# annegnx/PnP-Flow

Measured on AMD Instinct MI355X. Metric: restored images/sec, higher is better.
Workload: dtype f32-equivalent (f16 hi+lo split operands, 3 x f16 MFMA per product, f32 accumulate); 1 GPU; CelebA-shaped 256x256 box-inpainting (half-size 40, sigma 0.05) pnp_flow B=32/GPU 100x5 (the configuration BASELINE.json's metric is quoted on; main.py:132-136 at 256^2); image=256x256x3, batch_per_gpu=32, global_batch=32, steps_pnp=100, num_samples=5, weights=synthetic seed 0 (no checkpoint offline), hipgraph=True, unet_batch=160, parallelism=dp1 (contiguous shards of the global batch, no data-path collective)

## Files before the change

pnpflow_amd/csrc/conv_mfma16.hip:

```cpp
#include <cstdlib>
#include "pp_common.h"

namespace pf {

typedef float f32x16 __attribute__((ext_vector_type(16)));
typedef _Float16 f16x8 __attribute__((ext_vector_type(8)));
typedef _Float16 f16x4 __attribute__((ext_vector_type(4)));

__device__ __forceinline__ float silu_fast16(float x) { return x * __builtin_amdgcn_rcpf(1.0f + __expf(-x)); }

constexpr int conv16_lb(int MT, int WM, int KC) { return ((MT == 4 && WM == 2 && KC == 16) || (KC != 64 && ((MT == 4 && WM == 1) || (MT == 2 && WM == 4)))) ? 3 : 1; }

template <int MT, int NT, int WM, int WN, int S, int UP, int KC, bool GNB = false, int TERMS = 3>
__global__ __launch_bounds__(256, conv16_lb(MT, WM, KC)) void conv_mfma16_kernel(const ConvParams p) {
    constexpr int ROW = (TERMS == 3 ? KC : KC / 2) + 4;
    constexpr int KQ = KC / 4, KH = KC / 2, KS = KC / 16;
    constexpr int TH = 2 * MT * WM, TW = 16;
    constexpr int HALO = KC == 64 ? 0 : 1;
    constexpr int PH = (TH - 1) * S + 1 + 2 * HALO, PW = (TW - 1) * S + 1 + 2 * HALO, PP = PH * PW;
    constexpr int RS = ((PW * ROW + 63) / 64) * 64;
    constexpr int BN = WN * NT * 32;
    constexpr int A_F4 = PP * KQ, A_PER = (A_F4 + 255) / 256;
    static_assert(WM * WN == 4, "4 waves per workgroup");

    extern __shared__ __attribute__((aligned(16))) char smem_raw[];
    uint32_t* s_patch = reinterpret_cast<uint32_t*>(smem_raw);
    constexpr int EPI = 4 * 32 * 36 + WM * BN * 2;
    float* s_sc = reinterpret_cast<float*>(s_patch + (PH * RS > EPI ? PH * RS : EPI));
    float* s_sh = s_sc + ((p.gn_C + 3) & ~3);

    const int tiles_x = (p.W + TW - 1) / TW, tiles_y = (p.H + TH - 1) / TH;
    int bid, nb;
    if (p.xcd_map) {
        const int NBk = gridDim.y == 1 ? (p.Cout + BN - 1) / BN : 1;
        const int total = gridDim.x;
        const int work = (blockIdx.x & 7) * (total >> 3) + (blockIdx.x >> 3);
        bid = work / NBk; nb = work % NBk;
    } else {
        bid = blockIdx.x; nb = blockIdx.y;
    }
    const int tx = bid % tiles_x; bid /= tiles_x;
    const int ty = bid % tiles_y;
    const int b = bid / tiles_y;
    const int oy0 = ty * TH, ox0 = tx * TW, n0 = nb * BN;
    const int tid = threadIdx.x, lane = tid & 63, wave = tid >> 6, hi = lane >> 5, l31 = lane & 31;
    const int wm = wave % WM, wn = wave / WM;
    const int Hv = UP ? 2 * p.Hs : p.Hs, Wv = UP ? 2 * p.Ws : p.Ws;
    const int qi = tid % KQ, q4 = qi * 4;
    float seg_scale[3], seg_inv[3];
#pragma unroll
    for (int i = 0; i < 3; ++i) { seg_scale[i] = p.scale != nullptr ? p.scale[8 * b + i] : 1.0f; seg_inv[i] = p.scale != nullptr ? p.scale[8 * b + 4 + i] : 1.0f; }

    int a_pix[A_PER];
#pragma unroll
    for (int i = 0; i < A_PER; ++i) {
        const int idx = tid + i * 256;
        a_pix[i] = -1;
        if (idx < A_F4) {
            const int pix = idx / KQ;
            const int py = pix / PW, px = pix % PW;
            const int gy = oy0 * S - HALO + py, gx = ox0 * S - HALO + px;
            if (gy >= 0 && gy < Hv && gx >= 0 && gx < Wv && !(UP == 2 && ((gy | gx) & 1))) {
                const int sy = UP ? (gy >> 1) : gy, sx = UP ? (gx >> 1) : gx;
                a_pix[i] = (b * p.Hs + sy) * (p.src_row_pitch > 0 ? p.src_row_pitch : p.Ws) + sx;
            }
        }
    }

    float4 ra[A_PER];
    auto prefetch = [&](int si, int ch) {
        const ConvSeg& sg = p.seg[si];
        const int c = min(ch * KC + q4, sg.C - 4);
        const float* base = sg.src + sg.coff + c;
#pragma unroll
        for (int i = 0; i < A_PER; ++i) ra[i] = *reinterpret_cast<const float4*>(base + (size_t)max(a_pix[i], 0) * sg.cstride);
    };
    auto store_lds = [&](int si, int ch) {
        const ConvSeg& sg = p.seg[si];
        const int c = ch * KC + q4;
        const bool cok = c < sg.C;
        float4 sc = make_float4(1.f, 1.f, 1.f, 1.f), sh = make_float4(0.f, 0.f, 0.f, 0.f);
        if (sg.xform != 0 && cok) {
            sc = *reinterpret_cast<const float4*>(s_sc + sg.gn_off + c);
            sh = *reinterpret_cast<const float4*>(s_sh + sg.gn_off + c);
        }
        const float a_scale = si == 0 ? seg_scale[0] : (si == 1 ? seg_scale[1] : seg_scale[2]);
#pragma unroll
        for (int i = 0; i < A_PER; ++i) {
            if (tid + i * 256 < A_F4) {
                const int a_p = (tid + i * 256) / KQ;
                const int a_lds = (a_p / PW) * RS + (a_p % PW) * ROW + qi * 2;
                float4 v = ra[i];
                if (sg.xform != 0) {
                    v.x = v.x * sc.x + sh.x; v.y = v.y * sc.y + sh.y;
                    v.z = v.z * sc.z + sh.z; v.w = v.w * sc.w + sh.w;
                    if (sg.xform == 2) {
                        v.x = silu_fast16(v.x); v.y = silu_fast16(v.y); v.z = silu_fast16(v.z); v.w = silu_fast16(v.w);
                    }
                }
                v.x *= a_scale; v.y *= a_scale; v.z *= a_scale; v.w *= a_scale;
                if (!(cok && a_pix[i] >= 0)) v = make_float4(0.f, 0.f, 0.f, 0.f);
                if constexpr (TERMS == 3) {
                    uint2 h, l;
                    split4_pp(v, h.x, h.y, l.x, l.y);
                    *reinterpret_cast<uint2*>(s_patch + a_lds) = h;
                    *reinterpret_cast<uint2*>(s_patch + a_lds + KH) = l;
                } else {
                    f16x4 h;
                    h[0] = (_Float16)v.x; h[1] = (_Float16)v.y; h[2] = (_Float16)v.z; h[3] = (_Float16)v.w;
                    *reinterpret_cast<f16x4*>(s_patch + a_lds) = h;
                }
            }
        }
    };

    constexpr int GNP = 4;
    float csc[GNP], csh[GNP];
    {
        const float* cb = p.coef + (size_t)b * 2 * p.coef_stride;
#pragma unroll
        for (int i = 0; i < GNP; ++i) {
            csc[i] = 0.f; csh[i] = 0.f;
            if (i * 256 < p.gn_C) {
                const int c = min(tid + i * 256, p.gn_C - 1);
                csc[i] = cb[c]; csh[i] = cb[p.coef_stride + c];
            }
        }
    }
    prefetch(0, 0);
#pragma unroll
    for (int i = 0; i < GNP; ++i) {
        const int c = tid + i * 256;
        if (c < p.gn_C) { s_sc[c] = csc[i]; s_sh[c] = csh[i]; }
    }

    f32x16 acc[MT][NT];
#pragma unroll
    for (int mt = 0; mt < MT; ++mt)
#pragma unroll
        for (int nt = 0; nt < NT; ++nt)
#pragma unroll
            for (int r = 0; r < 16; ++r) acc[mt][nt][r] = 0.f;

    const int prow = l31 >> 4, pcol = l31 & 15;
    const int nbase = n0 + wn * NT * 32 + l31;
    int nclamp[NT];
#pragma unroll
    for (int nt = 0; nt < NT; ++nt) nclamp[nt] = min(nbase + nt * 32, p.Cout - 1);

    auto load_b = [&](const ConvSeg& sg, int ch, int s, uint4 (&dh)[NT], uint4 (&dl)[NT]) {
        const int tap = s / KS, j = s % KS;
        const size_t kidx = ((size_t)ch * KS + j) * sg.taps + tap;
        const uint4* wp = reinterpret_cast<const uint4*>(sg.w16) + kidx * ((size_t)p.Cout * 4) + hi;
#pragma unroll
        for (int nt = 0; nt < NT; ++nt) { dh[nt] = wp[(size_t)nclamp[nt] * 2]; if constexpr (TERMS == 3) dl[nt] = wp[(size_t)p.Cout * 2 + (size_t)nclamp[nt] * 2]; else dl[nt] = dh[nt]; }
    };

    int si = 0, ch = 0;
    while (true) {
        const ConvSeg& sg = p.seg[si];
        if (ch == 0 && si > 0) {
            const float ratio = (si == 1 ? seg_scale[1] * seg_inv[0] : seg_scale[2] * seg_inv[1]);
            if (ratio != 1.0f)
            {
#pragma unroll
                for (int mt = 0; mt < MT; ++mt)
#pragma unroll
                    for (int nt = 0; nt < NT; ++nt)
#pragma unroll
                        for (int r = 0; r < 16; ++r) acc[mt][nt][r] *= ratio;
            }
        }
        __syncthreads();
        store_lds(si, ch);
        __syncthreads();
        int nsi = si, nch = ch + 1;
        if (nch * KC >= sg.C) { nsi = si + 1; nch = 0; }
        const bool more = nsi < p.nseg;

        const int nsteps = sg.taps * KS;
        uint4 bh0[NT], bl0[NT], bh1[NT], bl1[NT], bh2[NT], bl2[NT];
        load_b(sg, ch, 0, bh0, bl0); load_b(sg, ch, min(1, nsteps - 1), bh1, bl1);
        if (more) prefetch(nsi, nch);

        auto k_step = [&](int s, uint4 (&ch_)[NT], uint4 (&cl_)[NT], uint4 (&nh_)[NT], uint4 (&nl_)[NT]) {
            load_b(sg, ch, min(s + 2, nsteps - 1), nh_, nl_);
            __builtin_amdgcn_sched_barrier(0);
            const int tap = s / KS, j = s % KS;
            const int ky = sg.taps == 9 ? tap / 3 : (sg.taps == 4 ? (tap >> 1) + sg.oy : HALO), kx = sg.taps == 9 ? tap % 3 : (sg.taps == 4 ? (tap & 1) + sg.ox : HALO);
            f16x8 ah[MT], al[MT];
#pragma unroll
            for (int mt = 0; mt < MT; ++mt) {
                const int poff = (((wm * MT + mt) * 2 + prow) * S + ky) * RS + (pcol * S + kx) * ROW;
                ah[mt] = *reinterpret_cast<const f16x8*>(s_patch + poff + j * 8 + hi * 4);
                if constexpr (TERMS == 3) al[mt] = *reinterpret_cast<const f16x8*>(s_patch + poff + KH + j * 8 + hi * 4); else al[mt] = ah[mt];
            }
            if constexpr (!(MT == 4 && WM == 1)) __builtin_amdgcn_sched_barrier(0);
            if constexpr (TERMS == 3) {
#pragma unroll
            for (int mt = 0; mt < MT; ++mt)
#pragma unroll
                for (int nt = 0; nt < NT; ++nt)
                    acc[mt][nt] = __builtin_amdgcn_mfma_f32_32x32x16_f16(al[mt], *reinterpret_cast<const f16x8*>(&ch_[nt]), acc[mt][nt], 0, 0, 0);
#pragma unroll
            for (int mt = 0; mt < MT; ++mt)
#pragma unroll
                for (int nt = 0; nt < NT; ++nt)
                    acc[mt][nt] = __builtin_amdgcn_mfma_f32_32x32x16_f16(ah[mt], *reinterpret_cast<const f16x8*>(&cl_[nt]), acc[mt][nt], 0, 0, 0);
            }
#pragma unroll
            for (int mt = 0; mt < MT; ++mt)
#pragma unroll
                for (int nt = 0; nt < NT; ++nt)
                    acc[mt][nt] = __builtin_amdgcn_mfma_f32_32x32x16_f16(ah[mt], *reinterpret_cast<const f16x8*>(&ch_[nt]), acc[mt][nt], 0, 0, 0);
        };
        __builtin_amdgcn_s_setprio(2);
        int s = 0;
        for (; s + 3 <= nsteps; s += 3) {
            k_step(s, bh0, bl0, bh2, bl2); k_step(s + 1, bh1, bl1, bh0, bl0); k_step(s + 2, bh2, bl2, bh1, bl1);
        }
        if (nsteps - s >= 1) k_step(s, bh0, bl0, bh2, bl2);
        if (nsteps - s == 2) k_step(s + 1, bh1, bl1, bh0, bl0);
        __builtin_amdgcn_s_setprio(0);
        if (!more) break;
        si = nsi; ch = nch;
    }

    __syncthreads();
    constexpr int TP = 36;
    float* s_tr = reinterpret_cast<float*>(s_patch) + wave * (32 * TP);
    float* s_red = reinterpret_cast<float*>(s_patch) + 4 * 32 * TP;
    const float oscale = p.out_scale * (1.0f / 256.0f) * (p.nseg == 1 ? seg_inv[0] : (p.nseg == 2 ? seg_inv[1] : seg_inv[2]));
    const int cq = lane & 7;
#pragma unroll
    for (int nt = 0; nt < NT; ++nt) {
        const int ncol = n0 + (wn * NT + nt) * 32;
        const int n = ncol + l31;
        const float add = (p.addvec != nullptr && n < p.Cout) ? p.addvec[(size_t)b * p.addvec_bs + n] : 0.f;
        const int n4 = ncol + cq * 4;
        const bool nok4 = n4 < p.Cout;
        float s1[4] = {0.f, 0.f, 0.f, 0.f}, s2[4] = {0.f, 0.f, 0.f, 0.f};
        float4 g_mu, g_rs, g_ga, g_be;
        if constexpr (GNB) {
            const int gc = p.gnb_coff + min(n4, p.Cout - 4);
            g_mu = *reinterpret_cast<const float4*>(p.gnb_mu + (size_t)b * p.gnb_Ct + gc);
            g_rs = *reinterpret_cast<const float4*>(p.gnb_rs + (size_t)b * p.gnb_Ct + gc);
            g_ga = *reinterpret_cast<const float4*>(p.gnb_gamma + gc);
            g_be = *reinterpret_cast<const float4*>(p.gnb_beta + gc);
        }
        constexpr int RG = (MT >= 2 && WN != 4) ? 2 : 1;
        float4 rv[RG][4];
        float4 xv[GNB ? RG : 1][4];
#pragma unroll
        for (int mt = 0; mt < MT; ++mt) {
            if constexpr (GNB) {
                if (mt % RG == 0) {
#pragma unroll
                    for (int g = 0; g < RG; ++g)
#pragma unroll
                        for (int i = 0; i < 4; ++i) {
                            const int px = (lane >> 3) + 8 * i;
                            const int oy = min(oy0 + (wm * MT + mt + g) * 2 + (px >> 4), p.H - 1), ox = min(ox0 + (px & 15), p.W - 1);
                            const size_t pix = ((size_t)b * p.H + oy) * p.W + ox;
                            xv[g][i] = *reinterpret_cast<const float4*>(p.gnb_x + pix * p.gnb_xstride + min(n4, p.Cout - 4));
                        }
                }
            }
            if (mt % RG == 0 && p.residual != nullptr) {
#pragma unroll
                for (int g = 0; g < RG; ++g)
#pragma unroll
                    for (int i = 0; i < 4; ++i) {
                        const int px = (lane >> 3) + 8 * i;
                        const int oy = min(oy0 + (wm * MT + mt + g) * 2 + (px >> 4), p.H - 1), ox = min(ox0 + (px & 15), p.W - 1);
                        const size_t pix = ((size_t)b * p.H + oy) * (p.dst_row_pitch > 0 ? p.dst_row_pitch : p.W) + ox;
                        rv[g][i] = *reinterpret_cast<const float4*>(p.residual + pix * p.res_cstride + min(n4, p.Cout - 4));
                    }
            }
#pragma unroll
            for (int r = 0; r < 16; ++r) {
                const int row = (r & 3) + 8 * (r >> 2) + 4 * hi;
                s_tr[row * TP + l31] = acc[mt][nt][r] * oscale + add;
            }
            __builtin_amdgcn_fence(__ATOMIC_RELEASE, "workgroup");
            __builtin_amdgcn_wave_barrier();
            __builtin_amdgcn_fence(__ATOMIC_ACQUIRE, "workgroup");
#pragma unroll
            for (int i = 0; i < 4; ++i) {
                const int px = (lane >> 3) + 8 * i;
                const int oy = oy0 + (wm * MT + mt) * 2 + (px >> 4), ox = ox0 + (px & 15);
                float4 v = *reinterpret_cast<const float4*>(s_tr + px * TP + cq * 4);
                if (nok4 && oy < p.H && ox < p.W) {
                    const size_t pix = ((size_t)b * p.H + oy) * (p.dst_row_pitch > 0 ? p.dst_row_pitch : p.W) + ox;
                    if (p.residual != nullptr) {
                        const float rsc = p.res_scale;
                        v.x = fmaf(rv[mt % RG][i].x, rsc, v.x); v.y = fmaf(rv[mt % RG][i].y, rsc, v.y); v.z = fmaf(rv[mt % RG][i].z, rsc, v.z); v.w = fmaf(rv[mt % RG][i].w, rsc, v.w);
                    }
                    if constexpr (GNB) {
                        const float4 xx = xv[mt % RG][i];
                        float d[4] = {v.x, v.y, v.z, v.w};
                        const float xs[4] = {xx.x, xx.y, xx.z, xx.w}, mm[4] = {g_mu.x, g_mu.y, g_mu.z, g_mu.w}, rr[4] = {g_rs.x, g_rs.y, g_rs.z, g_rs.w};
                        const float gg[4] = {g_ga.x, g_ga.y, g_ga.z, g_ga.w}, bb[4] = {g_be.x, g_be.y, g_be.z, g_be.w};
#pragma unroll
                        for (int j = 0; j < 4; ++j) {
                            const float yh = (xs[j] - mm[j]) * rr[j];
                            if (p.gnb_silu) {
                                const float u = yh * gg[j] + bb[j];
                                const float sg = __builtin_amdgcn_rcpf(1.0f + __expf(-u));
                                d[j] *= sg * (1.0f + u * (1.0f - sg));
                            }
                            d[j] *= gg[j];
                            s1[j] += d[j]; s2[j] += d[j] * yh;
                        }
                        *reinterpret_cast<float4*>(p.out + pix * p.out_cstride + n4) = make_float4(d[0], d[1], d[2], d[3]);
                    } else {
                    *reinterpret_cast<float4*>(p.out + pix * p.out_cstride + n4) = (p.pack_from_p1 != 0 && n4 >= p.pack_from_p1 - 1) ? pack_hilo4(v) : v;
                    s1[0] += v.x; s1[1] += v.y; s1[2] += v.z; s1[3] += v.w;
                    s2[0] += v.x * v.x; s2[1] += v.y * v.y; s2[2] += v.z * v.z; s2[3] += v.w * v.w;
                    }
                }
            }
            __builtin_amdgcn_fence(__ATOMIC_RELEASE, "workgroup");
            __builtin_amdgcn_wave_barrier();
            __builtin_amdgcn_fence(__ATOMIC_ACQUIRE, "workgroup");
        }
        if (GNB || p.stats_out != nullptr) {
#pragma unroll
            for (int j = 0; j < 4; ++j) {
#pragma unroll
                for (int o = 8; o < 64; o <<= 1) { s1[j] += __shfl_xor(s1[j], o); s2[j] += __shfl_xor(s2[j], o); }
            }
            if (lane < 8) {
#pragma unroll
                for (int j = 0; j < 4; ++j) {
                    const int col = (wn * NT + nt) * 32 + cq * 4 + j;
                    s_red[(wm * BN + col) * 2] = s1[j]; s_red[(wm * BN + col) * 2 + 1] = s2[j];
                }
            }
        }
    }
    if (GNB || p.stats_out != nullptr) {
        __syncthreads();
        for (int t = tid; t < BN * 2; t += 256) {
            const int col = t >> 1, which = t & 1;
            float tot = 0.f;
#pragma unroll
            for (int w = 0; w < WM; ++w) tot += s_red[(w * BN + col) * 2 + which];
            const int n = n0 + col;
            if (n < p.Cout) {
                if constexpr (GNB) unsafeAtomicAdd(p.gnb_sum + ((size_t)b * p.gnb_Ct + p.gnb_coff + n) * 2 + which, (double)tot);
                else unsafeAtomicAdd(p.stats_out + ((size_t)b * p.Cout + n) * 2 + which, (double)tot);
            }
        }
    }
}

template <int MT, int NT, int WM, int WN, int S, int UP, int KC, int TERMS>
static hipError_t launch_cfg16(const ConvParams& p, hipStream_t stream) {
    constexpr int ROW = (TERMS == 3 ? KC : KC / 2) + 4;
    constexpr int TH = 2 * MT * WM, TW = 16;
    constexpr int HALO = KC == 64 ? 0 : 1;
    constexpr int PH = (TH - 1) * S + 1 + 2 * HALO, PW = (TW - 1) * S + 1 + 2 * HALO;
    constexpr int RS = ((PW * ROW + 63) / 64) * 64;
    constexpr int BN = WN * NT * 32;
    constexpr int EPI = 4 * 32 * 36 + WM * BN * 2;
    const size_t lds = (size_t)((PH * RS > EPI ? PH * RS : EPI) + 2 * ((p.gn_C + 3) & ~3)) * 4;
    const int tiles = p.B * ((p.H + TH - 1) / TH) * ((p.W + TW - 1) / TW);
    dim3 grid(tiles, (p.Cout + BN - 1) / BN);
    ConvParams pp = p; pp.xcd_map = 0;
    if (((long)grid.x * grid.y) % 8 == 0) { pp.xcd_map = 1; grid = dim3(grid.x * grid.y, 1); }
    if constexpr (S == 1 && UP == 0) {
        if (p.gnb_x != nullptr) {
            static unsigned long long attr_set_g = 0ull;
            auto kg = conv_mfma16_kernel<MT, NT, WM, WN, S, UP, KC, true, TERMS>;
            { hipError_t e = set_max_dynamic_lds_once(reinterpret_cast<const void*>(kg), attr_set_g, 160 * 1024); if (e != hipSuccess) return e; }
            hipLaunchKernelGGL(kg, grid, dim3(256), lds, stream, pp);
            return hipGetLastError();
        }
    }
    if (p.gnb_x != nullptr) return hipErrorInvalidValue;
    static unsigned long long attr_set = 0ull;
    auto kern = conv_mfma16_kernel<MT, NT, WM, WN, S, UP, KC, false, TERMS>;
    { hipError_t e = set_max_dynamic_lds_once(reinterpret_cast<const void*>(kern), attr_set, 160 * 1024); if (e != hipSuccess) return e; }
    hipLaunchKernelGGL(kern, grid, dim3(256), lds, stream, pp);
    return hipGetLastError();
}

static long wg_count16(const ConvParams& p, int TH, int BN) {
    return (long)p.B * ((p.H + TH - 1) / TH) * ((p.W + 15) / 16) * ((p.Cout + BN - 1) / BN);
}

template <int S, int UP, int KC, int TERMS>
static hipError_t launch_sel16(const ConvParams& p, hipStream_t stream) {
    constexpr long MIN_WGS = KC == 64 ? 1024 : 512;
    if constexpr (S == 1) {
        if (p.Cout <= 32) {
            return launch_cfg16<2, 1, 4, 1, S, UP, KC, TERMS>(p, stream);
        }
        if (p.Cout <= 64) {
            if (wg_count16(p, 16, 64) >= MIN_WGS) return launch_cfg16<4, 1, 2, 2, S, UP, KC, TERMS>(p, stream);
            if (wg_count16(p, 8, 64) >= MIN_WGS) return launch_cfg16<2, 1, 2, 2, S, UP, KC, TERMS>(p, stream);
            return launch_cfg16<1, 1, 2, 2, S, UP, KC, TERMS>(p, stream);
        }
        if (wg_count16(p, 8, 128) >= MIN_WGS) return launch_cfg16<4, 1, 1, 4, S, UP, KC, TERMS>(p, stream);
        if (wg_count16(p, 4, 128) >= MIN_WGS) return launch_cfg16<2, 1, 1, 4, S, UP, KC, TERMS>(p, stream);
        return launch_cfg16<1, 1, 2, 2, S, UP, KC, TERMS>(p, stream);
    } else {
        if (p.Cout <= 32) return launch_cfg16<1, 1, 4, 1, S, UP, KC, TERMS>(p, stream);
        if (p.Cout <= 64) return launch_cfg16<2, 1, 2, 2, S, UP, KC, TERMS>(p, stream);
        return launch_cfg16<1, 1, 2, 2, S, UP, KC, TERMS>(p, stream);
    }
}

template <int TERMS>
static hipError_t launch_conv16_t(const ConvParams& p, int stride, int up, hipStream_t stream) {
    if (p.gn_C > 1024 || (p.gn_C > 0 && p.coef == nullptr)) return hipErrorInvalidValue;
    bool all_1tap = true;
    for (int i = 0; i < p.nseg; ++i) {
        if (p.seg[i].w_mode != 0 || p.seg[i].w16 == nullptr) return hipErrorInvalidValue;
        all_1tap &= p.seg[i].taps == 1 && p.seg[i].C % 64 == 0;
    }
    bool all32 = true;
    for (int i = 0; i < p.nseg; ++i) all32 &= p.seg[i].C % 32 == 0;
    if (all_1tap && stride == 1 && !up) return launch_sel16<1, 0, 64, TERMS>(p, stream);
    if (stride == 2) return launch_sel16<2, 0, 16, TERMS>(p, stream);
    if (up == 2) return launch_sel16<1, 2, 16, TERMS>(p, stream);
    if (up) return all32 ? launch_sel16<1, 1, 32, TERMS>(p, stream) : launch_sel16<1, 1, 16, TERMS>(p, stream);
    return all32 ? launch_sel16<1, 0, 32, TERMS>(p, stream) : launch_sel16<1, 0, 16, TERMS>(p, stream);
}

hipError_t launch_conv16(const ConvParams& p, int stride, int up, hipStream_t stream, int terms) {
    return terms == 1 ? launch_conv16_t<1>(p, stride, up, stream) : launch_conv16_t<3>(p, stride, up, stream);
}

}
```

Baseline: 3.328 images/s.

## Feed 1x1 shortcut segments directly from global memory into MFMA registers

Adds a DIRECT variant of the fp16-split conv kernel. After the 3x3 segment's chunks, the trailing one-tap (1x1 shortcut) segments are loaded straight from global memory into registers, split into hi/lo f16 and fed to MFMA, skipping the LDS staging and the per-chunk barriers. Loads run through a three-deep rotating register pipeline, and the launch bound rises to 2 for MT=4. It is gated by an env var that defaults on and applies to eligible stride-1, KC=32, NT=1, WM=2/WN=2 launches. The extra register buffers may hurt occupancy, and raw global loads lose LDS reuse.

```diff
diff --git a/pnpflow_amd/csrc/conv_mfma16.hip b/pnpflow_amd/csrc/conv_mfma16.hip
--- a/pnpflow_amd/csrc/conv_mfma16.hip
+++ b/pnpflow_amd/csrc/conv_mfma16.hip
@@ -1,4 +1,5 @@
 #include <cstdlib>
+#include <type_traits>
 #include "pp_common.h"
 
 namespace pf {
@@ -9,10 +10,11 @@
 
 __device__ __forceinline__ float silu_fast16(float x) { return x * __builtin_amdgcn_rcpf(1.0f + __expf(-x)); }
 
-constexpr int conv16_lb(int MT, int WM, int KC) { return ((MT == 4 && WM == 2 && KC == 16) || (KC != 64 && ((MT == 4 && WM == 1) || (MT == 2 && WM == 4)))) ? 3 : 1; }
-
-template <int MT, int NT, int WM, int WN, int S, int UP, int KC, bool GNB = false, int TERMS = 3>
-__global__ __launch_bounds__(256, conv16_lb(MT, WM, KC)) void conv_mfma16_kernel(const ConvParams p) {
+constexpr int conv16_lb(int MT, int WM, int KC, int DIRECT = 0) { return ((MT == 4 && WM == 2 && KC == 16) || (KC != 64 && ((MT == 4 && WM == 1) || (MT == 2 && WM == 4)))) ? 3 : (DIRECT != 0 && MT == 4 ? 2 : 1); }
+
+template <int MT, int NT, int WM, int WN, int S, int UP, int KC, bool GNB = false, int TERMS = 3, int DIRECT = 0>
+__global__ __launch_bounds__(256, conv16_lb(MT, WM, KC, DIRECT)) void conv_mfma16_kernel(const ConvParams p) {
+    static_assert(DIRECT == 0 || (S == 1 && UP == 0 && KC == 32 && !GNB), "direct one-tap segments: plain stride-1 launches with 32-channel chunks");
     constexpr int ROW = (TERMS == 3 ? KC : KC / 2) + 4;
     constexpr int KQ = KC / 4, KH = KC / 2, KS = KC / 16;
     constexpr int TH = 2 * MT * WM, TW = 16;
@@ -67,15 +69,16 @@
         }
     }
 
-    float4 ra[A_PER];
-    auto prefetch = [&](int si, int ch) {
+    constexpr int RW = 2 * MT;
+    float4 ra[DIRECT != 0 && A_PER < 2 * RW ? 2 * RW : A_PER];
+    auto prefetch = [&](int si, int ch) __attribute__((always_inline)) {
         const ConvSeg& sg = p.seg[si];
         const int c = min(ch * KC + q4, sg.C - 4);
         const float* base = sg.src + sg.coff + c;
 #pragma unroll
         for (int i = 0; i < A_PER; ++i) ra[i] = *reinterpret_cast<const float4*>(base + (size_t)max(a_pix[i], 0) * sg.cstride);
     };
-    auto store_lds = [&](int si, int ch) {
+    auto store_lds = [&](int si, int ch) __attribute__((always_inline)) {
         const ConvSeg& sg = p.seg[si];
         const int c = ch * KC + q4;
         const bool cok = c < sg.C;
@@ -84,7 +87,7 @@
             sc = *reinterpret_cast<const float4*>(s_sc + sg.gn_off + c);
             sh = *reinterpret_cast<const float4*>(s_sh + sg.gn_off + c);
         }
-        const float a_scale = si == 0 ? seg_scale[0] : (si == 1 ? seg_scale[1] : seg_scale[2]);
+        const float a_scale = (DIRECT != 0 || si == 0) ? seg_scale[0] : (si == 1 ? seg_scale[1] : seg_scale[2]);
 #pragma unroll
         for (int i = 0; i < A_PER; ++i) {
             if (tid + i * 256 < A_F4) {
@@ -148,16 +151,49 @@
 #pragma unroll
     for (int nt = 0; nt < NT; ++nt) nclamp[nt] = min(nbase + nt * 32, p.Cout - 1);
 
-    auto load_b = [&](const ConvSeg& sg, int ch, int s, uint4 (&dh)[NT], uint4 (&dl)[NT]) {
+    auto load_b_at = [&](const void* w16, size_t kidx, uint4 (&dh)[NT], uint4 (&dl)[NT]) __attribute__((always_inline)) {
+        const uint4* wp = reinterpret_cast<const uint4*>(w16) + kidx * ((size_t)p.Cout * 4) + hi;
+#pragma unroll
+        for (int nt = 0; nt < NT; ++nt) { dh[nt] = wp[(size_t)nclamp[nt] * 2]; if constexpr (TERMS == 3) dl[nt] = wp[(size_t)p.Cout * 2 + (size_t)nclamp[nt] * 2]; else dl[nt] = dh[nt]; }
+    };
+    auto load_b = [&](const ConvSeg& sg, int ch, int s, uint4 (&dh)[NT], uint4 (&dl)[NT]) __attribute__((always_inline)) {
         const int tap = s / KS, j = s % KS;
-        const size_t kidx = ((size_t)ch * KS + j) * sg.taps + tap;
-        const uint4* wp = reinterpret_cast<const uint4*>(sg.w16) + kidx * ((size_t)p.Cout * 4) + hi;
-#pragma unroll
-        for (int nt = 0; nt < NT; ++nt) { dh[nt] = wp[(size_t)nclamp[nt] * 2]; if constexpr (TERMS == 3) dl[nt] = wp[(size_t)p.Cout * 2 + (size_t)nclamp[nt] * 2]; else dl[nt] = dh[nt]; }
-    };
-
-    int si = 0, ch = 0;
-    while (true) {
+        load_b_at(sg.w16, ((size_t)ch * KS + j) * sg.taps + tap, dh, dl);
+    };
+
+    int d_lsi = 0, d_lc = 0, d_ln = 0, d_lcs = 0;
+    const float* d_lsrc = nullptr; const void* d_lw16 = nullptr;
+    auto d_next = [&]() __attribute__((always_inline)) {
+        if (d_lc + 1 < d_ln) { d_lc += 1; }
+        else if (d_lsi + 1 < p.nseg) {
+            d_lsi += 1; d_lc = 0;
+            const ConvSeg& g = p.seg[d_lsi];
+            d_lsrc = g.src + g.coff; d_lw16 = g.w16; d_ln = g.C >> 4; d_lcs = g.cstride;
+        }
+    };
+    int d_pix[DIRECT ? MT : 1]; bool d_ok[DIRECT ? MT : 1];
+    if constexpr (DIRECT != 0) {
+#pragma unroll
+        for (int mt = 0; mt < MT; ++mt) {
+            const int oy = oy0 + (wm * MT + mt) * 2 + prow, ox = ox0 + pcol;
+            d_ok[mt] = oy < p.H && ox < p.W;
+            d_pix[mt] = (b * p.Hs + min(oy, p.H - 1)) * p.Ws + min(ox, p.W - 1);
+        }
+    }
+    auto load_raw = [&](float4* r, const float* src, int cs, int c) __attribute__((always_inline)) {
+        const float* base = src + c * 16 + hi * 8;
+#pragma unroll
+        for (int mt = 0; mt < (DIRECT ? MT : 1); ++mt) {
+            const float* q = base + (size_t)d_pix[mt] * cs;
+            r[2 * mt] = *reinterpret_cast<const float4*>(q); r[2 * mt + 1] = *reinterpret_cast<const float4*>(q + 4);
+        }
+    };
+    float4 rw2s[DIRECT ? RW : 1];
+    float4* const rw0 = ra; float4* const rw1 = ra + (DIRECT ? RW : 0); float4* const rw2 = rw2s;
+
+    uint4 bh0[NT], bl0[NT], bh1[NT], bl1[NT], bh2[NT], bl2[NT];
+    auto chunk = [&](int si, int ch, int& nsi, int& nch, bool& more, auto last_c) __attribute__((always_inline)) {
+        constexpr bool LAST = decltype(last_c)::value;
         const ConvSeg& sg = p.seg[si];
         if (ch == 0 && si > 0) {
             const float ratio = (si == 1 ? seg_scale[1] * seg_inv[0] : seg_scale[2] * seg_inv[1]);
@@ -174,17 +210,26 @@
         __syncthreads();
         store_lds(si, ch);
         __syncthreads();
-        int nsi = si, nch = ch + 1;
+        nsi = si; nch = ch + 1;
         if (nch * KC >= sg.C) { nsi = si + 1; nch = 0; }
-        const bool more = nsi < p.nseg;
+        more = DIRECT != 0 ? nsi == 0 : nsi < p.nseg;
 
         const int nsteps = sg.taps * KS;
-        uint4 bh0[NT], bl0[NT], bh1[NT], bl1[NT], bh2[NT], bl2[NT];
         load_b(sg, ch, 0, bh0, bl0); load_b(sg, ch, min(1, nsteps - 1), bh1, bl1);
-        if (more) prefetch(nsi, nch);
-
-        auto k_step = [&](int s, uint4 (&ch_)[NT], uint4 (&cl_)[NT], uint4 (&nh_)[NT], uint4 (&nl_)[NT]) {
-            load_b(sg, ch, min(s + 2, nsteps - 1), nh_, nl_);
+        if constexpr (!LAST) {
+            if (more) prefetch(nsi, nch);
+        } else {
+            const ConvSeg& g = p.seg[1]; load_raw(rw0, g.src + g.coff, g.cstride, 0); load_raw(rw1, g.src + g.coff, g.cstride, 1);
+        }
+
+        auto k_step = [&](int s, uint4 (&ch_)[NT], uint4 (&cl_)[NT], uint4 (&nh_)[NT], uint4 (&nl_)[NT]) __attribute__((always_inline)) {
+            if constexpr (LAST) {
+                const bool dw = s + 2 >= nsteps;
+                const int ls = min(s + 2, nsteps - 1);
+                load_b_at(dw ? p.seg[1].w16 : sg.w16, dw ? (size_t)(s + 2 - nsteps) : ((size_t)ch * KS + ls % KS) * sg.taps + ls / KS, nh_, nl_);
+            } else {
+                load_b(sg, ch, min(s + 2, nsteps - 1), nh_, nl_);
+            }
             __builtin_amdgcn_sched_barrier(0);
             const int tap = s / KS, j = s % KS;
             const int ky = sg.taps == 9 ? tap / 3 : (sg.taps == 4 ? (tap >> 1) + sg.oy : HALO), kx = sg.taps == 9 ? tap % 3 : (sg.taps == 4 ? (tap & 1) + sg.ox : HALO);
@@ -222,8 +267,92 @@
         if (nsteps - s >= 1) k_step(s, bh0, bl0, bh2, bl2);
         if (nsteps - s == 2) k_step(s + 1, bh1, bl1, bh0, bl0);
         __builtin_amdgcn_s_setprio(0);
-        if (!more) break;
-        si = nsi; ch = nch;
+    };
+    if constexpr (DIRECT == 0) {
+        int si = 0, ch = 0;
+        while (true) {
+            int nsi, nch; bool more;
+            chunk(si, ch, nsi, nch, more, std::false_type{});
+            if (!more) break;
+            si = nsi; ch = nch;
+        }
+    } else {
+        const int nch0 = p.seg[0].C / KC;
+        int nsi, nch; bool more;
+        for (int ch = 0; ch + 1 < nch0; ++ch) chunk(0, ch, nsi, nch, more, std::false_type{});
+        chunk(0, nch0 - 1, nsi, nch, more, std::true_type{});
+    }
+
+    if constexpr (DIRECT != 0) {
+        int nd = 0;
+        for (int i = 1; i < p.nseg; ++i) nd += p.seg[i].C >> 4;
+        int d_si = 1, d_c = 0, d_n = p.seg[1].C >> 4;
+        d_next(); d_next(); d_next();
+        auto d_step = [&](const float4* cr, uint4 (&ch_)[NT], uint4 (&cl_)[NT], float4* nr, uint4 (&nh_)[NT], uint4 (&nl_)[NT]) __attribute__((always_inline)) {
+            load_raw(nr, d_lsrc, d_lcs, d_lc);
+            load_b_at(d_lw16, (size_t)d_lc, nh_, nl_);
+            d_next();
+            __builtin_amdgcn_sched_barrier(0);
+            if (d_c == 0) {
+                const float ratio = (d_si == 1 ? seg_scale[1] * seg_inv[0] : seg_scale[2] * seg_inv[1]);
+                if (ratio != 1.0f) {
+#pragma unroll
+                    for (int mt = 0; mt < MT; ++mt)
+#pragma unroll
+                        for (int nt = 0; nt < NT; ++nt)
+#pragma unroll
+                            for (int r = 0; r < 16; ++r) acc[mt][nt][r] *= ratio;
+                }
+            }
+            const float a_scale = d_si == 1 ? seg_scale[1] : seg_scale[2];
+            f16x8 ah[MT], al[MT];
+#pragma unroll
+            for (int mt = 0; mt < MT; ++mt) {
+                const float sc = d_ok[mt] ? a_scale : 0.f;
+                float4 v0 = cr[2 * mt], v1 = cr[2 * mt + 1];
+                v0.x *= sc; v0.y *= sc; v0.z *= sc; v0.w *= sc; v1.x *= sc; v1.y *= sc; v1.z *= sc; v1.w *= sc;
+                if constexpr (TERMS == 3) {
+                    uint4 h, l;
+                    split4_pp(v0, h.x, h.y, l.x, l.y); split4_pp(v1, h.z, h.w, l.z, l.w);
+                    ah[mt] = __builtin_bit_cast(f16x8, h); al[mt] = __builtin_bit_cast(f16x8, l);
+                } else {
+                    f16x8 h;
+                    h[0] = (_Float16)v0.x; h[1] = (_Float16)v0.y; h[2] = (_Float16)v0.z; h[3] = (_Float16)v0.w;
+                    h[4] = (_Float16)v1.x; h[5] = (_Float16)v1.y; h[6] = (_Float16)v1.z; h[7] = (_Float16)v1.w;
+                    ah[mt] = h; al[mt] = h;
+                }
+            }
+            if constexpr (TERMS == 3) {
+#pragma unroll
+            for (int mt = 0; mt < MT; ++mt)
+#pragma unroll
+                for (int nt = 0; nt < NT; ++nt)
+                    acc[mt][nt] = __builtin_amdgcn_mfma_f32_32x32x16_f16(al[mt], *reinterpret_cast<const f16x8*>(&ch_[nt]), acc[mt][nt], 0, 0, 0);
+#pragma unroll
+            for (int mt = 0; mt < MT; ++mt)
+#pragma unroll
+                for (int nt = 0; nt < NT; ++nt)
+                    acc[mt][nt] = __builtin_amdgcn_mfma_f32_32x32x16_f16(ah[mt], *reinterpret_cast<const f16x8*>(&cl_[nt]), acc[mt][nt], 0, 0, 0);
+            }
+#pragma unroll
+            for (int mt = 0; mt < MT; ++mt)
+#pragma unroll
+                for (int nt = 0; nt < NT; ++nt)
+                    acc[mt][nt] = __builtin_amdgcn_mfma_f32_32x32x16_f16(ah[mt], *reinterpret_cast<const f16x8*>(&ch_[nt]), acc[mt][nt], 0, 0, 0);
+            if (d_c + 1 < d_n) { d_c += 1; }
+            else if (d_si + 1 < p.nseg) { d_si += 1; d_c = 0; d_n = p.seg[d_si].C >> 4; }
+        };
+        __builtin_amdgcn_s_setprio(2);
+        int s = 0;
+        if (nd >= 3) {
+            d_step(rw0, bh0, bl0, rw2, bh2, bl2); d_step(rw1, bh1, bl1, rw0, bh0, bl0); d_step(rw2, bh2, bl2, rw1, bh1, bl1);
+            for (s = 3; s + 3 <= nd; s += 3) {
+                d_step(rw0, bh0, bl0, rw2, bh2, bl2); d_step(rw1, bh1, bl1, rw0, bh0, bl0); d_step(rw2, bh2, bl2, rw1, bh1, bl1);
+            }
+        }
+        if (nd - s >= 1) d_step(rw0, bh0, bl0, rw2, bh2, bl2);
+        if (nd - s == 2) d_step(rw1, bh1, bl1, rw0, bh0, bl0);
+        __builtin_amdgcn_s_setprio(0);
     }
 
     __syncthreads();
@@ -353,6 +482,15 @@
             }
         }
     }
+}
+
+static int conv16_direct_mode() { static const int mode = getenv("PNPFLOW_HIP_C16_DIRECT") ? atoi(getenv("PNPFLOW_HIP_C16_DIRECT")) : 1; return mode; }
+
+static bool conv16_direct_ok(const ConvParams& p) {
+    if (conv16_direct_mode() == 0 || p.nseg < 2 || p.gnb_x != nullptr || p.src_row_pitch > 0 || p.seg[0].taps != 9) return false;
+    for (int i = 1; i < p.nseg; ++i)
+        if (p.seg[i].taps != 1 || p.seg[i].xform != 0 || p.seg[i].C % 32 != 0 || p.seg[i].cstride % 4 != 0 || p.seg[i].coff % 4 != 0) return false;
+    return true;
 }
 
 template <int MT, int NT, int WM, int WN, int S, int UP, int KC, int TERMS>
@@ -379,6 +517,15 @@
         }
     }
     if (p.gnb_x != nullptr) return hipErrorInvalidValue;
+    if constexpr (S == 1 && UP == 0 && KC == 32 && NT == 1 && WM == 2 && WN == 2) {
+        if (conv16_direct_ok(p)) {
+            static unsigned long long attr_set_d = 0ull;
+            auto kd = conv_mfma16_kernel<MT, NT, WM, WN, S, UP, KC, false, TERMS, 1>;
+            { hipError_t e = set_max_dynamic_lds_once(reinterpret_cast<const void*>(kd), attr_set_d, 160 * 1024); if (e != hipSuccess) return e; }
+            hipLaunchKernelGGL(kd, grid, dim3(256), lds, stream, pp);
+            return hipGetLastError();
+        }
+    }
     static unsigned long long attr_set = 0ull;
     auto kern = conv_mfma16_kernel<MT, NT, WM, WN, S, UP, KC, false, TERMS>;
     { hipError_t e = set_max_dynamic_lds_once(reinterpret_cast<const void*>(kern), attr_set, 160 * 1024); if (e != hipSuccess) return e; }
```

After: 3.316 images/s. Within noise of the previous version (-0.4%).
